# nibox/Pose-Estimation-with-Message-Passing-Networks

Hardware: AMD Instinct MI355X
Metric: images/sec (640px, HRNet-w48) + MPN edge-updates/sec at 1/2/4/8 MI355X (higher is better)
Workload: dtype f16x3; 1 GPU; c3: 8x17x640x640 heatmaps/GPU -> fully graph -> MPN TypeAware-attn T=3; images_per_gpu=8, global_batch=8, persons_per_image=9, nodes_per_gpu=1224, edges_per_gpu=186048, parallelism=image-sharded x1, batches_in_flight=2, detection_and_node_math=fp32

## Files before the change

include/pemp.h:

```cpp
#ifndef PEMP_H_
#define PEMP_H_

#include <stddef.h>
#include <stdint.h>

#ifdef __cplusplus
extern "C" {
#endif

#define PEMP_ABI_VERSION 24

enum {
  PEMP_OK = 0,
  PEMP_ERR_INVALID_ARG = -1,
  PEMP_ERR_HIP = -2,
  PEMP_ERR_WORKSPACE = -3,
  PEMP_ERR_UNSUPPORTED = -4,
};

int pemp_abi_version(void);
const char* pemp_last_error(void);
int pemp_device_check(void);

enum { PEMP_DETECT_NMS = 1, PEMP_DETECT_SELECT = 2, PEMP_DETECT_ALL = 3 };
// ... 174 lines not shown
  const float* edge_img;
  const uint16_t* emb_comp_bf;
  const float* emb_comp_b;
} pemp_mpn_weights;

typedef struct pemp_mpn_desc {
  int32_t num_types;
  int32_t num_joints;
  int32_t steps;
  int32_t aux_loss_steps;
  int32_t aggr;
  int32_t hidden;
  int32_t edge_attr_dim;
  int32_t node_in_dim;
  int32_t precision;
  int32_t types_stride;
  int32_t flags;
} pemp_mpn_desc;

#define PEMP_MPN_PREPARED 1
#define PEMP_MPN_TWO_LAUNCH_FIRST 4
#define PEMP_MPN_FUSED_FIRST_PROFILED 8
#define PEMP_MPN_SEPARATE_PRELUDE 16

size_t pemp_mpn_workspace_size(const pemp_mpn_desc* desc, int64_t N, int64_t E);
size_t pemp_mpn_fused_first_lds_bytes(void);
int pemp_mpn_prelude_grids(int64_t N, int64_t E, int B, int T, int nmax, int edge_grid, int cus, int32_t* out8);
int pemp_mpn_forward(const pemp_mpn_desc* desc, const pemp_mpn_weights* weights, const float* x,
                     const float* edge_attr, const int64_t* edge_index, const int64_t* node_types,
                     int64_t N, int64_t E, float* edge_logits, float* node_logits, float* class_logits,
                     void* workspace, size_t workspace_bytes, void* stream);

int pemp_mpn_forward_fully(const pemp_mpn_desc* desc, const pemp_mpn_weights* weights, const float* x,
                           const float* edge_attr, const int64_t* edge_index, const int64_t* node_types,
                           int64_t N, int64_t E, const int64_t* node_off, const int64_t* node_off_host, int B,
                           float* edge_logits, float* node_logits, float* class_logits,
                           void* workspace, size_t workspace_bytes, void* stream);

int pemp_mpn_forward_fully_cap(const pemp_mpn_desc* desc, const pemp_mpn_weights* weights, const float* x,
                               const float* edge_attr, const int64_t* node_types, int64_t n_cap, int64_t e_cap,
                               const int32_t* n_det, int det_cap, const int64_t* node_off, int B,
                               float* edge_logits, float* node_logits, float* class_logits,
                               void* workspace, size_t workspace_bytes, void* stream);

enum {
  PEMP_STEP_DET = 0, PEMP_STEP_DSC, PEMP_STEP_NDET, PEMP_STEP_X, PEMP_STEP_JDET, PEMP_STEP_JSC, PEMP_STEP_BIDX,
  PEMP_STEP_JTAGS, PEMP_STEP_EIDX, PEMP_STEP_EATTR, PEMP_STEP_NOFF, PEMP_STEP_LOGITS, PEMP_STEP_NOUT
};
typedef struct pemp_step_plan {
  int32_t B, J, H, W, pool_kernel, use_threshold, topk, det_cap, projected;
// ... 99 lines not shown
```

pose-estimation-with-message-passing-networks_amd/_lib.py:

```python
import ctypes
import threading
import os

LIB_PATH = os.environ.get("PEMP_LIB") or os.path.join(os.path.dirname(os.path.abspath(__file__)), "csrc",
                                                     "libpemp.so")
ABI_VERSION = 24

ERR_INVALID_ARG, ERR_HIP, ERR_WORKSPACE, ERR_UNSUPPORTED = -1, -2, -3, -4
MPN_PREPARED, MPN_TWO_LAUNCH_FIRST, MPN_FUSED_FIRST_PROFILED = 1, 4, 8
MPN_SEPARATE_PRELUDE = 16

c_i32, c_i64, c_f32, c_sz, c_p = ctypes.c_int32, ctypes.c_int64, ctypes.c_float, ctypes.c_size_t, ctypes.c_void_p


class PempLayer(ctypes.Structure):
    _fields_ = [("w", c_p), ("b", c_p), ("in_dim", c_i32), ("out_dim", c_i32), ("relu", c_i32), ("pad_", c_i32)]


class PempMlp(ctypes.Structure):
    _fields_ = [("layer", PempLayer * 4), ("n_layers", c_i32), ("pad_", c_i32)]


class PempMpnWeights(ctypes.Structure):
    _fields_ = [("node_emb", PempMlp), ("edge_emb", PempMlp),
                ("pre_w", c_p), ("pre_b", c_p), ("q0_w", c_p), ("q0_b", c_p), ("e1_w", c_p),
                ("e2_w", c_p), ("e2_b", c_p), ("msg_w", c_p), ("attn_w", c_p), ("upd_w", c_p), ("upd_b", c_p),
                ("edge_head", PempMlp), ("node_head", PempMlp), ("class_head", PempMlp),
                ("attn_b", c_f32), ("pad_", c_i32),
                ("e1_bf", c_p), ("e2_bf", c_p), ("msg_bf", c_p), ("head_bf", c_p), ("emb_bf", c_p),
                ("upd_bf", c_p), ("pre_bf", c_p), ("node_img", c_p), ("attn_bv", c_p),
                ("upd_mlp", PempMlp),
                ("ept_l1_w", c_p), ("ept_l1_b", c_p), ("ept_l2_w", c_p), ("ept_l2_b", c_p), ("ept_o1_w", c_p),
                ("ept_o2_w", c_p), ("edge_img", c_p), ("emb_comp_bf", c_p), ("emb_comp_b", c_p)]
# ... 42 lines not shown
                                           c_i64, c_i64, c_f32, c_i32, c_p, c_p, c_p, c_p, c_p, c_p, c_p, c_p, c_p]),
    "pemp_fully_graph": (c_i32, [c_p, c_p, c_i32, c_i64, c_p, c_p]),
    "pemp_knn_workspace_size": (c_sz, [c_p, c_i32]),
    "pemp_knn_graph_build": (c_i32, [c_p, c_p, c_p, c_i32, c_i32, c_p, c_sz, c_i64, c_p, c_p, c_p, c_i32, c_p,
                                     c_i32, c_f32, c_i32, c_p, c_p]),
    "pemp_feature_knn_workspace_size": (c_sz, [c_p, c_i32]),
    "pemp_knn_rows_layout": (c_i32, [c_p, c_i32, c_i32, c_p]),
    "pemp_feature_knn_graph_build": (c_i32, [c_p, c_i32, c_p, c_p, c_p, c_i32, c_i32, c_p, c_sz, c_i64, c_p, c_p,
                                             c_p, c_i32, c_p, c_i32, c_f32, c_i32, c_p, c_p]),
    "pemp_score_graph_workspace_size": (c_sz, [c_p, c_i32, c_i32]),
    "pemp_score_graph": (c_i32, [c_p, c_p, c_p, c_i32, c_i32, c_i64, c_p, c_sz, c_p, c_p]),
    "pemp_gather_projected": (c_i32, [c_p, c_p, c_p, c_i32, c_i32, c_i32, c_i32, c_f32, c_p, c_p, c_i64, c_p, c_p]),
    "pemp_gather_projected_conv": (c_i32, [c_p, c_p, c_p, c_i32, c_i32, c_p, c_p, c_i32, c_i32, c_i32, c_i32, c_i32,
                                           c_f32, c_p, c_p, c_i64, c_p, c_p]),
    "pemp_detect_projected": (c_i32, [c_p, c_p, c_i32, c_i32, c_i32, c_i32, c_i32, c_f32, c_i32, c_i32, c_i32, c_p,
                                      c_sz, c_p, c_p, c_p, c_i32, c_p, c_p]),
    "pemp_gather_projected_tags": (c_i32, [c_p, c_i32, c_i32, c_i32, c_i32, c_p, c_p, c_i64, c_p, c_p]),
    "pemp_project_maps": (c_i32, [c_p, c_i32, c_i32, c_i32, c_i32, c_i32, c_p, c_p, c_p]),
    "pemp_stage_merge": (c_i32, [c_p, c_i32, c_i32, c_i32, c_p, c_i32, c_i32, c_i32, c_i32, c_i32, c_p, c_p]),
    "pemp_edge_features": (c_i32, [c_p, c_p, c_i32, c_p, c_p, c_i64, c_i32, c_f32, c_i32, c_p, c_p]),
    "pemp_mpn_workspace_size": (c_sz, [ctypes.POINTER(PempMpnDesc), c_i64, c_i64]),
    "pemp_mpn_fused_first_lds_bytes": (c_sz, []),
    "pemp_mpn_prelude_grids": (c_i32, [c_i64, c_i64, c_i32, c_i32, c_i32, c_i32, c_i32, c_p]),
    "pemp_mpn_forward": (c_i32, [ctypes.POINTER(PempMpnDesc), ctypes.POINTER(PempMpnWeights), c_p, c_p, c_p, c_p,
                                 c_i64, c_i64, c_p, c_p, c_p, c_p, c_sz, c_p]),
    "pemp_mpn_forward_fully": (c_i32, [ctypes.POINTER(PempMpnDesc), ctypes.POINTER(PempMpnWeights), c_p, c_p, c_p,
                                       c_p, c_i64, c_i64, c_p, c_p, c_i32, c_p, c_p, c_p, c_p, c_sz, c_p]),
    "pemp_mpn_forward_fully_cap": (c_i32, [ctypes.POINTER(PempMpnDesc), ctypes.POINTER(PempMpnWeights), c_p, c_p,
                                           c_p, c_i64, c_i64, c_p, c_i32, c_p, c_i32, c_p, c_p, c_p, c_p, c_sz, c_p]),
    "pemp_mpn_graph_stats": (c_i32, [c_p]),
    "pemp_edge_cus_policy": (c_i32, [c_i32, c_i64, c_i32]),
    "pemp_abi_struct_size": (c_sz, [c_i32]),
    "pemp_mpn_forward_sym": (c_i32, [ctypes.POINTER(PempMpnDesc), ctypes.POINTER(PempMpnWeights), c_p, c_p, c_p,
                                     c_p, c_i64, c_i64, c_p, c_p, c_p, c_p, c_sz, c_p]),
    "pemp_mpn_forward_knn": (c_i32, [ctypes.POINTER(PempMpnDesc), ctypes.POINTER(PempMpnWeights), c_p, c_p, c_p,
                                     c_p, c_i64, c_i64, c_p, c_p, c_p, c_p, c_p, c_i32, c_p, c_p, c_p, c_p, c_sz,
                                     c_p]),
    "pemp_mpn_prepare": (c_i32, [ctypes.POINTER(PempMpnDesc), c_p, c_p, c_i64, c_i64, c_p, c_sz, c_p]),
    "pemp_mpn_order_layout": (c_i32, [ctypes.POINTER(PempMpnDesc), c_i64, c_i64, c_p]),
    "pemp_mpn_edge_image_floats": (c_sz, [ctypes.POINTER(PempMpnDesc), ctypes.POINTER(PempMpnWeights)]),
    "pemp_mpn_edge_image": (c_i32, [ctypes.POINTER(PempMpnDesc), ctypes.POINTER(PempMpnWeights), c_p, c_sz, c_p]),
    "pemp_mpn_node_image_floats": (c_sz, [ctypes.POINTER(PempMpnWeights)]),
    "pemp_mpn_node_image": (c_i32, [ctypes.POINTER(PempMpnWeights), c_p, c_sz, c_p]),
    "pemp_mpn_status": (c_i32, [ctypes.POINTER(PempMpnDesc), c_i64, c_i64, c_p, c_p]),
    "pemp_pose_edge_weights": (c_i32, [c_p, c_i64, c_p, c_p, c_f32, c_i32, c_p, c_i32, c_i64, c_i32, c_p, c_p, c_p,
                                       c_p]),
# ... 121 lines not shown
```

pose-estimation-with-message-passing-networks_amd/csrc/mpn.hip:

```cpp
#include <limits.h>

#include <algorithm>
#include <atomic>
#include <type_traits>
#include <map>
#include <mutex>
#include <string>
#include <vector>
#include <string.h>
#include <math.h>

#include "pemp_common.h"

namespace pemp {
namespace {

constexpr int D = 64;
constexpr int LDW = 72;
constexpr int MAXT = 17;
constexpr int EDGE_WAVES = 16;
constexpr int EMB_WAVES = 16, EMB_PER_CU = 1;
constexpr int EMB_MIN_WAVES_EU = EMB_WAVES * EMB_PER_CU / 4 > 1 ? EMB_WAVES * EMB_PER_CU / 4 : 1;
constexpr int RESERVE_CUS_DEFAULT = 64;
constexpr int64_t RESERVE_MIN_EDGES = 65536;
// ... 2441 lines not shown
          }
        }
    }
  }
}

__global__ __launch_bounds__(256) void node_rows_kernel(NodeRowsArgs a) {
  extern __shared__ __attribute__((aligned(16))) float lds[];
  node_rows_role(a, lds, blockIdx.x);
}

struct NodeTableArgs {
  const float* X;
  int64_t N;
  const float *pre_w, *pre_b;
  const uint16_t* pre_bf;
  int NO, groups;
  float* NT;
  const int64_t* ne;
  const float* agg;
  const int* seg;
  int T;
  const float* upd_b;
};

constexpr int64_t NODE_SUM_TABLE_MAX_MB = 16;
constexpr int TBL_TILES = 2;

template <int PREC, int TILES, bool SUM>
__device__ __forceinline__ void node_table_role(const NodeTableArgs& a, float* xs, int bx) {
  static_assert(!SUM || TILES == 1, "the summing variant takes one 16-node tile per workgroup");
  const int lane = threadIdx.x & 63, wave = threadIdx.x >> 6, c = lane & 15, g = lane >> 4;
  const int chunk = bx / a.groups, grp = bx - chunk * a.groups;
  const int64_t n0 = (int64_t)chunk * 16 * TILES, N = a.ne ? a.ne[0] : a.N;
  if (n0 >= N) return;
  const int nob = a.NO / 16, ob = grp * 4 + wave, obc = min(ob, nob - 1);
  float4 w[8];
  bf16x8_t wh[4], wlo[4];
  f16x8_t fh[4], flo[4];
  if (PREC == 0) {
#pragma unroll
    for (int mb = 0; mb < 8; ++mb) w[mb] = ld4(a.pre_w + (int64_t)(16 * obc + c) * 128 + 16 * mb + 4 * g);
  } else {
#pragma unroll
    for (int kb = 0; kb < 4; ++kb) {
      const int64_t o = (int64_t)(16 * obc + c) * 128 + 32 * kb + 8 * g;
      if (PREC == 1) {
        const __bf16* Wb = reinterpret_cast<const __bf16*>(a.pre_bf);
        wh[kb] = *reinterpret_cast<const bf16x8_t*>(Wb + o);
        wlo[kb] = *reinterpret_cast<const bf16x8_t*>(Wb + (int64_t)a.NO * 128 + o);
      } else {
        const _Float16* Wh = reinterpret_cast<const _Float16*>(a.pre_bf);
        fh[kb] = *reinterpret_cast<const f16x8_t*>(Wh + o);
        flo[kb] = *reinterpret_cast<const f16x8_t*>(Wh + (int64_t)a.NO * 128 + o);
      }
    }
  }
  const float4 bb = ld4(a.pre_b + 16 * obc + 4 * g);
  if constexpr (SUM) {
    const int r = threadIdx.x >> 4, q = threadIdx.x & 15;
    const int64_t n = n0 + r, nc = n < N ? n : N - 1;
    const int T = a.T;
    const float4 x0 = ld4(a.X + nc * 128 + 4 * q);
    float4 y[MAXT];
    int s0[MAXT], s1[MAXT];
#pragma unroll
    for (int t = 0; t < MAXT; ++t) {
      const int tc = min(t, T - 1);
      y[t] = ld4(a.agg + (nc * T + tc) * D + 4 * q);
      s0[t] = a.seg[tc * N + nc];
      s1[t] = a.seg[tc * N + nc + 1];
    }
    float4 v = ld4(a.upd_b + 4 * q);
#pragma unroll
    for (int t = 0; t < MAXT; ++t) {
      if (t < T && s1[t] > s0[t]) { v.x += y[t].x; v.y += y[t].y; v.z += y[t].z; v.w += y[t].w; }
    }
    v = make_float4(fmaxf(v.x, 0.f), fmaxf(v.y, 0.f), fmaxf(v.z, 0.f), fmaxf(v.w, 0.f));
    *reinterpret_cast<float4*>(&xs[r * RS + 4 * q]) = x0;
    *reinterpret_cast<float4*>(&xs[r * RS + 64 + 4 * q]) = v;
    if (grp == 0 && n < N) *reinterpret_cast<float4*>(const_cast<float*>(a.X) + n * 128 + 64 + 4 * q) = v;
  } else {
    float4 t[2 * TILES];
#pragma unroll
    for (int k = 0; k < 2 * TILES; ++k) {
      const int idx = threadIdx.x + 256 * k, row = idx >> 5, c4 = (idx & 31) * 4;
      const int64_t nn = min(n0 + row, N - 1);
      t[k] = ld4(a.X + nn * 128 + c4);
    }
    __builtin_amdgcn_sched_barrier(0);
#pragma unroll
    for (int k = 0; k < 2 * TILES; ++k) {
      const int idx = threadIdx.x + 256 * k, row = idx >> 5, c4 = (idx & 31) * 4;
      *reinterpret_cast<float4*>(&xs[row * RS + c4]) = t[k];
    }
  }
  __syncthreads();
  if (ob >= nob) return;
#pragma unroll
  for (int tile = 0; tile < TILES; ++tile) {
    const int64_t nn = n0 + 16 * tile + c;
    if (n0 + 16 * tile >= N) break;
    float x[8][4];
#pragma unroll
    for (int mb = 0; mb < 8; ++mb) {
// ... 36 lines not shown
#pragma unroll
        for (int kb = 0; kb < 2; ++kb) {
          uint32_t hw[4], lw[4];
#pragma unroll
          for (int d = 0; d < 4; ++d)
            split_pair(xh[2 * kb + (d >> 1)][2 * (d & 1)], xh[2 * kb + (d >> 1)][2 * (d & 1) + 1], ss, hw[d], lw[d]);
          const u32x4_t hv = {hw[0], hw[1], hw[2], hw[3]}, lv = {lw[0], lw[1], lw[2], lw[3]};
          hi[kb] = __builtin_bit_cast(f16x8_t, hv);
          lo[kb] = __builtin_bit_cast(f16x8_t, lv);
        }
#pragma unroll
        for (int kb = 0; kb < 2; ++kb) {
          acc = __builtin_amdgcn_mfma_f32_16x16x32_f16(flo[2 * h + kb], hi[kb], acc, 0, 0, 0);
          acc = __builtin_amdgcn_mfma_f32_16x16x32_f16(fh[2 * h + kb], lo[kb], acc, 0, 0, 0);
          acc = __builtin_amdgcn_mfma_f32_16x16x32_f16(fh[2 * h + kb], hi[kb], acc, 0, 0, 0);
        }
      }
      if (big) acc *= 1.0f / ss;
    }
    if (nn < N) st4(a.NT + nn * a.NO + 16 * ob + 4 * g, acc[0], acc[1], acc[2], acc[3]);
  }
}

template <int PREC, int TILES = TBL_TILES, bool SUM = false>
__global__ __launch_bounds__(256) void node_table_kernel(NodeTableArgs a) {
  __shared__ __attribute__((aligned(16))) float xs[16 * TILES * RS];
  node_table_role<PREC, TILES, SUM>(a, xs, blockIdx.x);
}

template <int PREC>
__global__ __launch_bounds__(256) void prelude_b_kernel(EdgeRangesArgs ra, NodeTableArgs ta, int split) {
  __shared__ __attribute__((aligned(16))) float xs[16 * TBL_TILES * RS];
  const int bx = blockIdx.x;
  if (bx < split) edge_ranges_role(ra, bx);
  else node_table_role<PREC, TBL_TILES, false>(ta, xs, bx - split);
}

static int grid1d(int64_t total, int block, int cap = 65536) {
  int64_t g = (total + block - 1) / block;
  return (int)(g < 1 ? 1 : (g > cap ? cap : g));
}

static bool published_head(const pemp_mlp& m) {
  return m.n_layers == 3 && m.layer[0].in_dim == 64 && m.layer[0].out_dim == 64 && m.layer[0].relu &&
         m.layer[1].in_dim == 64 && m.layer[1].out_dim == 32 && m.layer[1].relu && m.layer[2].in_dim == 32 &&
         m.layer[2].out_dim == 1 && !m.layer[2].relu;
}

template <int AGG, int PREC, int UPD, int STAGE>
static void launch_edge_step_s(const EdgeStepArgs& a, bool head, bool pub, int grid, hipStream_t st) {
  if (!head)
    hipLaunchKernelGGL((edge_step_kernel<AGG, 0, PREC, UPD, STAGE>), dim3(grid), dim3(64 * edge_waves<0>()), 0, st, a);
  else if (pub)
    hipLaunchKernelGGL((edge_step_kernel<AGG, 1, PREC, UPD, STAGE>), dim3(grid), dim3(64 * edge_waves_s<1, STAGE>()), 0,
                       st, a);
  else
    hipLaunchKernelGGL((edge_step_kernel<AGG, 2, PREC, UPD, STAGE>), dim3(grid), dim3(64 * edge_waves<2>()), 0, st, a);
}
// ... 865 lines not shown
  int rows_blocks;
  int a_split;
  int ranges_rb, ranges_blocks;
  int table_blocks;
  int b_split;
};

static PreludeGrids prelude_grids(int64_t N, int64_t E, int B, int T, int nmax, int G, int cus) {
  PreludeGrids g{};
  g.prep_gx = (int)std::max<int64_t>(1, std::min<int64_t>(64, ((int64_t)T * nmax * FULLY_PARTS + 511) / 512));
  g.rows_blocks = (int)((N + 15) / 16);
  g.a_gx = B > 0 ? std::max(1, std::min(g.prep_gx, (cus - g.rows_blocks) / B)) : g.prep_gx;
  g.a_split = g.a_gx * B;
  if (E > 0) {
    g.ranges_rb = std::min(64, (G * (EDGE_WAVES + 12) + 255) / 256);
    g.ranges_blocks = g.ranges_rb + (int)std::min<int64_t>(1024, (E + 255) / 256);
  }
  const int groups = ((128 + 64 * T) / 16 + 3) / 4;
  g.table_blocks = (int)(((N + 16 * TBL_TILES - 1) / (16 * TBL_TILES)) * groups);
  g.b_split = g.ranges_blocks;
  return g;
}

struct ForwardPlan {
  int T, J, steps, aux;
  int64_t tstride;
  bool upd_fused;
  bool pub_head;
  bool ept;
  bool emb_lds, emb_generic, comp, fixed;
  int emb_prec;
  EmbedLayout emb_lo;
  bool fused_heads, fused_embed;
  int edge_grid;
  int NO, table_prec, table_groups;
  unsigned node_grid, table_grid, table_grid1;
  int node_mode;
  bool sum_in_table;
  bool fused_first;
  PreludeGrids grids;
  bool paired;
};

static ForwardPlan plan_forward(const ForwardCall& c) {
  const pemp_mpn_desc& d = *c.desc;
  const pemp_mpn_weights& w = *c.w;
  const int64_t N = c.N, E = c.E;
  ForwardPlan p{};
  p.T = d.num_types; p.J = d.num_joints; p.steps = d.steps; p.aux = d.aux_loss_steps;
  p.tstride = d.types_stride > 0 ? d.types_stride : 1;
  p.upd_fused = edge_upd_fused(d, w);
  p.pub_head = edge_pub_head(d, w);
  p.ept = w.ept_l1_w != nullptr;
  p.emb_lds = mlp_ok(w.edge_emb, 64, 64);
  p.emb_prec = embed_prec(d, w);
  p.emb_lo = embed_layout(w.edge_emb, p.emb_prec);
  p.emb_generic = p.emb_lds && !embed_fixed_shape(p.emb_prec == PEMP_PREC_FP32
                                                      ? embed_layout(w.edge_emb, PEMP_PREC_F16X3)
                                                      : p.emb_lo);
  p.fixed = embed_fixed_shape(p.emb_lo);
  p.comp = embed_composed(p.emb_lo, p.emb_prec, w);
  p.fused_heads = node_heads_fused(w);
  p.fused_embed = node_embed_fused(w);
  p.edge_grid = std::max(edge_cus(E), p.T);
  p.NO = 128 + 64 * p.T;
  p.table_prec = d.precision != PEMP_PREC_FP32 && w.pre_bf ? d.precision : PEMP_PREC_FP32;
  p.table_groups = (p.NO / 16 + 3) / 4;
  p.grids = prelude_grids(N, E, c.order.kind == EdgeOrder::FULLY ? c.order.B : 0, p.T, c.order.nmax, p.edge_grid,
                          num_cus());
  p.node_grid = (unsigned)p.grids.rows_blocks;
  p.table_grid = (unsigned)p.grids.table_blocks;
  p.table_grid1 = (unsigned)(((N + 15) / 16) * p.table_groups);
  p.node_mode = p.upd_fused ? ROWS_SUM : (w.upd_w || w.upd_mlp.n_layers > 0) ? NODE_UPDATE_MLP : ROWS_COPY;
  p.sum_in_table = !p.ept && N * p.T * 256 * (int64_t)p.table_groups <= NODE_SUM_TABLE_MAX_MB << 20;
  p.fused_first = E > 0 && p.steps >= 2 && p.steps - p.aux - 1 > 0 && !(d.flags & PEMP_MPN_TWO_LAUNCH_FIRST) &&
                  d.precision == PEMP_PREC_F16X3 && d.aggr == PEMP_AGGR_ATTN && p.upd_fused && !p.ept &&
                  p.emb_lds && p.comp && w.edge_img &&
                  prof_repeat("edge_step") == 1 &&
                  (!prof_active() || (d.flags & PEMP_MPN_FUSED_FIRST_PROFILED));
  p.paired = c.order.kind == EdgeOrder::FULLY && !(d.flags & (PEMP_MPN_PREPARED | PEMP_MPN_SEPARATE_PRELUDE)) &&
             p.fused_embed && p.steps >= 1 && !prof_active();
  return p;
}

struct Forward {
  const ForwardCall& c;
  const ForwardPlan& p;
  const MpnWs ws;
  const hipStream_t st;
  const int64_t* ne = nullptr;
  const float* node_img = nullptr;
  const float* eimg = nullptr;
  float* r_cur;
  float* r_next;
  int rec = 0;

  Forward(const ForwardCall& call, const ForwardPlan& plan)
// ... 137 lines not shown

  int launch_paired() {
    const PreludeGrids& g = p.grids;
    const FullyPrepArgs fa = fully_args();
    const NodeRowsArgs na = rows_args(ROWS_EMBED, -1, false);
    hipLaunchKernelGGL(prelude_a_kernel, dim3((unsigned)(g.a_split + g.rows_blocks)), dim3(256),
                       prelude_a_lds_bytes(na), st, fa, na, g.a_split, g.a_gx);
    PEMP_LAUNCH_CHECK();
    const EdgeRangesArgs ra = ranges_args();
    const NodeTableArgs ta = table_args();
    with_prec(p.table_prec, [&](auto P) {
      hipLaunchKernelGGL(prelude_b_kernel<decltype(P)::value>, dim3((unsigned)(g.b_split + g.table_blocks)), dim3(256),
                         0, st, ra, ta, g.b_split);
    });
    PEMP_LAUNCH_CHECK();
    return PEMP_OK;
  }

  int node_step(int mode, bool table, int slot, bool dup) {
    const pemp_mpn_weights& w = *c.w;
    const int64_t N = c.N;
    const int T = p.T, J = p.J;
    if (mode == ROWS_SUM && table && slot < 0 && p.sum_in_table) {
      NodeTableArgs ta{ws.X, N, w.pre_w, w.pre_b, w.pre_bf, p.NO, p.table_groups, ws.NT, ne, ws.agg, ws.seg, T,
                       w.upd_b};
      ProfScope prof("node_update_table", st);
      with_prec(p.table_prec, [&](auto P) {
        hipLaunchKernelGGL((node_table_kernel<decltype(P)::value, 1, true>), dim3(p.table_grid1), dim3(256), 0, st, ta);
      });
      PEMP_LAUNCH_CHECK();
      return PEMP_OK;
    }
    if (mode == NODE_UPDATE_MLP && w.upd_mlp.n_layers > 0) {
      NodeMlpArgs ma{ws.agg, ws.seg, T, N, w.upd_mlp, nmlp_max_out(w.upd_mlp), ws.X, ne};
      ProfScope prof("node_update", st);
      hipLaunchKernelGGL(node_mlp_kernel, dim3(p.node_grid), dim3(256), nmlp_lds_bytes(T, w.upd_mlp), st, ma);
      PEMP_LAUNCH_CHECK();
      mode = ROWS_NONE;
    } else if (mode == NODE_UPDATE_MLP) {
      NodeUpdateArgs ua{ws.agg, ws.seg, T, N, w.upd_w, w.upd_b, ws.X, ne};
      ProfScope prof("node_update", st);
      hipLaunchKernelGGL(node_update_kernel, dim3(p.node_grid, 4), dim3(64 * UPD_WAVES), 0, st, ua);
      PEMP_LAUNCH_CHECK();
      mode = ROWS_NONE;
    }
    const NodeRowsArgs na = rows_args(mode, slot, dup);
    if (na.mode != ROWS_NONE || na.node_out) {
      ProfScope prof(mode == ROWS_EMBED ? "node_embed" : "node_update", st);
      hipLaunchKernelGGL(node_rows_kernel, dim3(p.node_grid), dim3(256), node_rows_lds_bytes(na), st, na);
      PEMP_LAUNCH_CHECK();
    }
// ... 379 lines not shown
                        as_stream(stream));
}

extern "C" int pemp_mpn_order_layout(const pemp_mpn_desc* desc, int64_t N, int64_t E, size_t* offs) {
  PEMP_CHECK_ARG(desc && offs && desc->num_types >= 1 && desc->num_types <= MAXT, "pemp_mpn_order_layout: bad desc");
  PEMP_CHECK_ARG(N >= 0 && E >= 0, "pemp_mpn_order_layout: N=%lld E=%lld out of range", (long long)N, (long long)E);
  mpn_carve(nullptr, desc->num_types, N, E, nullptr, offs);
  return PEMP_OK;
}

extern "C" size_t pemp_mpn_fused_first_lds_bytes(void) { return edge_first_lds_bytes(); }

extern "C" int pemp_mpn_prelude_grids(int64_t N, int64_t E, int B, int T, int nmax, int edge_grid, int cus,
                                      int32_t* out8) {
  PEMP_CHECK_ARG(out8 && N >= 0 && E >= 0 && B >= 0 && B <= FULLY_MAXB && T >= 1 && T <= MAXT && nmax >= 0 &&
                     nmax <= FULLY_MAXN && edge_grid >= 1 && cus >= 1,
                 "pemp_mpn_prelude_grids: bad args");
  const PreludeGrids g = prelude_grids(N, E, B, T, nmax, edge_grid, cus);
  static_assert(sizeof(PreludeGrids) == 8 * sizeof(int32_t), "eight ints");
  memcpy(out8, &g, sizeof(g));
  return PEMP_OK;
}

extern "C" size_t pemp_mpn_edge_image_floats(const pemp_mpn_desc* desc, const pemp_mpn_weights* w) {
  if (!desc || !w || desc->num_types < 1 || desc->num_types > MAXT) return 0;
  if (!mlp_ok(w->edge_emb, 64, 64)) return edge_image_base_floats(*desc, *w);
  return embed_image_offset(*desc, *w) + embed_image_floats(embed_layout(w->edge_emb, embed_prec(*desc, *w)));
}

extern "C" int pemp_mpn_edge_image(const pemp_mpn_desc* desc, const pemp_mpn_weights* w, float* image, size_t floats,
                                   void* stream) {
  PEMP_CHECK_ARG(desc && w && image, "pemp_mpn_edge_image: null pointer");
  PEMP_CHECK_ARG(desc->num_types >= 1 && desc->num_types <= MAXT, "pemp_mpn_edge_image: bad num_types");
  PEMP_CHECK_ARG(desc->precision == PEMP_PREC_FP32 || (w->e1_bf && w->e2_bf && w->msg_bf),
                 "pemp_mpn_edge_image: split precisions need the *_bf packs");
  PEMP_CHECK_ARG(w->e1_w && w->e2_w && w->e2_b && w->msg_w, "pemp_mpn_edge_image: null layer weights");
  PEMP_CHECK_ARG(desc->aggr != PEMP_AGGR_ATTN || w->attn_w, "pemp_mpn_edge_image: attention needs attn_w");
  const size_t need = pemp_mpn_edge_image_floats(desc, w);
  PEMP_CHECK_ARG(floats >= need, "pemp_mpn_edge_image: image needs %zu floats", need);
  EdgeImgArgs ia = edge_image_args(*desc, *w, edge_upd_fused(*desc, *w), edge_pub_head(*desc, *w), image);
  hipLaunchKernelGGL(edge_image_kernel, dim3(16, (unsigned)desc->num_types), dim3(256), 0, as_stream(stream), ia);
  PEMP_LAUNCH_CHECK();
  if (mlp_ok(w->edge_emb, 64, 64)) {
    const int prec = embed_prec(*desc, *w);
    const EmbedLayout lo = embed_layout(w->edge_emb, prec);
    float* eimg = image + embed_image_offset(*desc, *w);
// ... 52 lines not shown
```

pose-estimation-with-message-passing-networks_amd/mpn/model.py:

```python
import ctypes
import itertools
import os
import warnings

import numpy as np
import torch
import torch.nn as nn

from .. import _lib
from .fold import F16RangeError, fold_weights
from .edge_type import TypeAwareEdgeUpdate
from .hierarch import HierarchUpdateCnn, HierarchUpdateMlp

_VALIDATE = os.environ.get("PEMP_VALIDATE", "0") not in ("", "0")
_DEBUG_SYNC = os.environ.get("PEMP_DEBUG_SYNC", "0") not in ("", "0")
_FULLY_OFF = os.environ.get("PEMP_NO_FULLY_PREPARE", "0") not in ("", "0")
_SYM_OFF = os.environ.get("PEMP_NO_SYM_PREPARE", "0") not in ("", "0")
_KNN_OFF = os.environ.get("PEMP_NO_KNN_PREPARE", "0") not in ("", "0")
_EDGE_LIMIT = (1 << 23) - 1

AGGR_CODES = {"attn": 0, "add": 1, "sum": 1, "mean": 2, "max": 3}
PRECISIONS = {"fp32": 0, "bf16x3": 1, "f16x3": 2}


def default_precision(aggr_code):
    env = os.environ.get("PEMP_PRECISION", "")
    if env:
        if env not in PRECISIONS:
            raise ValueError(f"PEMP_PRECISION={env!r}: expected one of {sorted(PRECISIONS)}")
        return env
    return "f16x3"
TYPE_LUTS = {"left_right": [0, 1, 1, 2, 2, 3, 3, 4, 4, 5, 5, 6, 6, 7, 7, 8, 8],
             "per_body_part": [0, 0, 0, 0, 0, 1, 1, 2, 3, 2, 3, 4, 5, 4, 5, 4, 5]}


def _rows(logits, n):
    L = logits.shape[1]
    if L != 1:
        return list((logits if logits.shape[0] == n else logits[:n]).unbind(0))
    return [logits[r].view(L, 1).squeeze() for r in range(n)]

# ... 148 lines not shown
        self.node_classification = _make_mlp(64, config.NODE_CLASS.OUTPUT_SIZES, bn=config.BN)
        self.classification = _make_mlp(64, config.CLASS.OUTPUT_SIZES, bn=config.BN)
        self.edge_steps = config.STEPS
        self.node_steps = config.NODE_STEPS
        self.aux_loss_steps = config.AUX_LOSS_STEPS
        self.num_joints = config.CLASS.OUTPUT_SIZES[-1]
        if self.node_steps != 0:
            raise NotImplementedError("NODE_STEPS > 0 (the reference calls the layer without node_types)")
        if config.AGGR_TYPE == "per_type":
            aggr = "attn" if config.AGGR_SUB in ("node_edge_attn", "node_edge_attn_per_type") else config.AGGR
        else:
            aggr = config.AGGR
        if aggr not in AGGR_CODES:
            raise NotImplementedError(f"AGGR={aggr}")
        self.aggr_code = AGGR_CODES[aggr]
        self.precision = default_precision(self.aggr_code)
        self._folded = None
        self._folded_key = None
        self._tensors = None
        self._ws = _lib.Workspace()
        self._desc_ent = None
        self.fuse_first_pass = None
        self.paired_prelude = True
        self.fused_edge_update = False
        self._cap_ok = True
        self._edge_limit = _EDGE_LIMIT
        self._node_rows_limit = _EDGE_LIMIT

    def _apply(self, fn, *args, **kwargs):
        self._tensors = None
        self._folded = None
        return super()._apply(fn, *args, **kwargs)

    def _load_from_state_dict(self, *args, **kwargs):
        self._tensors = None
        return super()._load_from_state_dict(*args, **kwargs)

    def _weights(self, device):
        if self._tensors is None:
            self._tensors = list(self.parameters()) + list(self.buffers())
        key = (device, self.precision, [t._version for t in self._tensors])
        if self._folded is None or self._folded_key != key:
            try:
                self._folded = fold_weights(self, device, self.precision)
            except F16RangeError as exc:
                warnings.warn(f"{exc}; this model runs in precision 'fp32'")
                self.precision = "fp32"
                key = (device, self.precision, key[2])
                self._folded = fold_weights(self, device, self.precision)
            self._folded_key = key
        return self._folded

    def _first_flag(self):
        f = self.fuse_first_pass
        first = 0 if f is None else _lib.MPN_FUSED_FIRST_PROFILED if f else _lib.MPN_TWO_LAUNCH_FIRST
        return first | (0 if self.paired_prelude else _lib.MPN_SEPARATE_PRELUDE)

    def _descriptor(self, A, C, t_stride):
        dkey = (A, C, self.precision, t_stride, self.fuse_first_pass, self.paired_prelude)
        ent = self._desc_ent
        if ent is None or ent[0] != dkey:
            steps, aux = self.edge_steps, self.aux_loss_steps
            self._n_rec = sum(1 for i in range(steps) if i >= steps - aux - 1)
            desc = _lib.PempMpnDesc(self.num_types, self.num_joints, steps, aux, self.aggr_code, 64, A, C,
                                    PRECISIONS[self.precision], t_stride, self._first_flag())
            ent = self._desc_ent = (dkey, ctypes.byref(desc))
        return ent[1]

    _desc_ref = property(lambda self: self._desc_ent[1])
    _desc = property(lambda self: self._desc_ent[1]._obj)

    def _forward_blocks(self, x, edge_attr, edge_index, node_types, kwargs):
        dev = x.device
        N, E = x.shape[0], edge_index.shape[1]
        ei = edge_index.long()
        lo = torch.minimum(ei[0], ei[1])
        blocks = node_blocks(ei, N, self._edge_limit, self._node_rows_limit // self.num_types)
        n_rec = sum(1 for i in range(self.edge_steps) if i >= self.edge_steps - self.aux_loss_steps - 1)
        edge_logits = torch.empty(max(n_rec, 1), E, dtype=torch.float32, device=dev)
        node_logits = torch.empty(n_rec + 1, N, dtype=torch.float32, device=dev)
        class_logits = torch.empty(n_rec + 1, N, self.num_joints, dtype=torch.float32, device=dev)
        sub_kw = {k: v for k, v in kwargs.items() if k == "validate"}
# ... 178 lines not shown
```

Baseline: 36530 images/s.

## Add dedicated node-sum table kernel with weight prefetch and split precision fragments

Replaces the SUM variant of the node table role with a dedicated kernel. It sums per-type aggregates, builds the split hi/lo precision fragments once into LDS, then loops over several output groups per workgroup while prefetching the next group's weight fragment. A grid planner picks tiles per workgroup and groups per run so the grid still covers the CUs, and the segment-emptiness checks are turned into a ballot bitmask. Env flags can force the fused or separate node step. This cuts redundant per-node aggregate loads and fragment conversions across output groups, at the cost of more register and LDS pressure and fewer workgroups.

```diff
diff --git a/include/pemp.h b/include/pemp.h
--- a/include/pemp.h
+++ b/include/pemp.h
@@ -220,10 +220,13 @@
 #define PEMP_MPN_TWO_LAUNCH_FIRST 4
 #define PEMP_MPN_FUSED_FIRST_PROFILED 8
 #define PEMP_MPN_SEPARATE_PRELUDE 16
+#define PEMP_MPN_SEPARATE_NODE_STEP 32
+#define PEMP_MPN_FUSED_NODE_STEP 64
 
 size_t pemp_mpn_workspace_size(const pemp_mpn_desc* desc, int64_t N, int64_t E);
 size_t pemp_mpn_fused_first_lds_bytes(void);
 int pemp_mpn_prelude_grids(int64_t N, int64_t E, int B, int T, int nmax, int edge_grid, int cus, int32_t* out8);
+int pemp_mpn_node_step_grid(int64_t N, int T, int cus, int32_t* out4);
 int pemp_mpn_forward(const pemp_mpn_desc* desc, const pemp_mpn_weights* weights, const float* x,
                      const float* edge_attr, const int64_t* edge_index, const int64_t* node_types,
                      int64_t N, int64_t E, float* edge_logits, float* node_logits, float* class_logits,
diff --git a/pose-estimation-with-message-passing-networks_amd/_lib.py b/pose-estimation-with-message-passing-networks_amd/_lib.py
--- a/pose-estimation-with-message-passing-networks_amd/_lib.py
+++ b/pose-estimation-with-message-passing-networks_amd/_lib.py
@@ -9,6 +9,7 @@
 ERR_INVALID_ARG, ERR_HIP, ERR_WORKSPACE, ERR_UNSUPPORTED = -1, -2, -3, -4
 MPN_PREPARED, MPN_TWO_LAUNCH_FIRST, MPN_FUSED_FIRST_PROFILED = 1, 4, 8
 MPN_SEPARATE_PRELUDE = 16
+MPN_SEPARATE_NODE_STEP, MPN_FUSED_NODE_STEP = 32, 64
 
 c_i32, c_i64, c_f32, c_sz, c_p = ctypes.c_int32, ctypes.c_int64, ctypes.c_float, ctypes.c_size_t, ctypes.c_void_p
 
@@ -97,6 +98,7 @@
     "pemp_mpn_workspace_size": (c_sz, [ctypes.POINTER(PempMpnDesc), c_i64, c_i64]),
     "pemp_mpn_fused_first_lds_bytes": (c_sz, []),
     "pemp_mpn_prelude_grids": (c_i32, [c_i64, c_i64, c_i32, c_i32, c_i32, c_i32, c_i32, c_p]),
+    "pemp_mpn_node_step_grid": (c_i32, [c_i64, c_i32, c_i32, c_p]),
     "pemp_mpn_forward": (c_i32, [ctypes.POINTER(PempMpnDesc), ctypes.POINTER(PempMpnWeights), c_p, c_p, c_p, c_p,
                                  c_i64, c_i64, c_p, c_p, c_p, c_p, c_sz, c_p]),
     "pemp_mpn_forward_fully": (c_i32, [ctypes.POINTER(PempMpnDesc), ctypes.POINTER(PempMpnWeights), c_p, c_p, c_p,
diff --git a/pose-estimation-with-message-passing-networks_amd/csrc/mpn.hip b/pose-estimation-with-message-passing-networks_amd/csrc/mpn.hip
--- a/pose-estimation-with-message-passing-networks_amd/csrc/mpn.hip
+++ b/pose-estimation-with-message-passing-networks_amd/csrc/mpn.hip
@@ -2487,65 +2487,64 @@
   const int* seg;
   int T;
   const float* upd_b;
+  int runs, G;
 };
 
 constexpr int64_t NODE_SUM_TABLE_MAX_MB = 16;
 constexpr int TBL_TILES = 2;
 
-template <int PREC, int TILES, bool SUM>
+template <int PREC>
+struct TableFrag {
+  u32x4_t hi[4], lo[4];
+  float4 bb;
+};
+template <>
+struct TableFrag<0> {
+  float4 w[8];
+  float4 bb;
+};
+
+template <int PREC>
+__device__ __forceinline__ TableFrag<PREC> table_frag_load(const NodeTableArgs& a, int ob, int c, int g) {
+  TableFrag<PREC> f;
+  if constexpr (PREC == 0) {
+#pragma unroll
+    for (int mb = 0; mb < 8; ++mb) f.w[mb] = ld4(a.pre_w + (int64_t)(16 * ob + c) * 128 + 16 * mb + 4 * g);
+  } else {
+#pragma unroll
+    for (int kb = 0; kb < 4; ++kb) {
+      const uint16_t* o = a.pre_bf + (int64_t)(16 * ob + c) * 128 + 32 * kb + 8 * g;
+      f.hi[kb] = *reinterpret_cast<const u32x4_t*>(o);
+      f.lo[kb] = *reinterpret_cast<const u32x4_t*>(o + (int64_t)a.NO * 128);
+    }
+  }
+  f.bb = ld4(a.pre_b + 16 * ob + 4 * g);
+  return f;
+}
+
+template <int PREC, int TILES>
 __device__ __forceinline__ void node_table_role(const NodeTableArgs& a, float* xs, int bx) {
-  static_assert(!SUM || TILES == 1, "the summing variant takes one 16-node tile per workgroup");
   const int lane = threadIdx.x & 63, wave = threadIdx.x >> 6, c = lane & 15, g = lane >> 4;
   const int chunk = bx / a.groups, grp = bx - chunk * a.groups;
   const int64_t n0 = (int64_t)chunk * 16 * TILES, N = a.ne ? a.ne[0] : a.N;
   if (n0 >= N) return;
   const int nob = a.NO / 16, ob = grp * 4 + wave, obc = min(ob, nob - 1);
+  const TableFrag<PREC> f = table_frag_load<PREC>(a, obc, c, g);
   float4 w[8];
   bf16x8_t wh[4], wlo[4];
   f16x8_t fh[4], flo[4];
-  if (PREC == 0) {
-#pragma unroll
-    for (int mb = 0; mb < 8; ++mb) w[mb] = ld4(a.pre_w + (int64_t)(16 * obc + c) * 128 + 16 * mb + 4 * g);
+  if constexpr (PREC == 0) {
+#pragma unroll
+    for (int mb = 0; mb < 8; ++mb) w[mb] = f.w[mb];
   } else {
 #pragma unroll
     for (int kb = 0; kb < 4; ++kb) {
-      const int64_t o = (int64_t)(16 * obc + c) * 128 + 32 * kb + 8 * g;
-      if (PREC == 1) {
-        const __bf16* Wb = reinterpret_cast<const __bf16*>(a.pre_bf);
-        wh[kb] = *reinterpret_cast<const bf16x8_t*>(Wb + o);
-        wlo[kb] = *reinterpret_cast<const bf16x8_t*>(Wb + (int64_t)a.NO * 128 + o);
-      } else {
-        const _Float16* Wh = reinterpret_cast<const _Float16*>(a.pre_bf);
-        fh[kb] = *reinterpret_cast<const f16x8_t*>(Wh + o);
-        flo[kb] = *reinterpret_cast<const f16x8_t*>(Wh + (int64_t)a.NO * 128 + o);
-      }
-    }
-  }
-  const float4 bb = ld4(a.pre_b + 16 * obc + 4 * g);
-  if constexpr (SUM) {
-    const int r = threadIdx.x >> 4, q = threadIdx.x & 15;
-    const int64_t n = n0 + r, nc = n < N ? n : N - 1;
-    const int T = a.T;
-    const float4 x0 = ld4(a.X + nc * 128 + 4 * q);
-    float4 y[MAXT];
-    int s0[MAXT], s1[MAXT];
-#pragma unroll
-    for (int t = 0; t < MAXT; ++t) {
-      const int tc = min(t, T - 1);
-      y[t] = ld4(a.agg + (nc * T + tc) * D + 4 * q);
-      s0[t] = a.seg[tc * N + nc];
-      s1[t] = a.seg[tc * N + nc + 1];
-    }
-    float4 v = ld4(a.upd_b + 4 * q);
-#pragma unroll
-    for (int t = 0; t < MAXT; ++t) {
-      if (t < T && s1[t] > s0[t]) { v.x += y[t].x; v.y += y[t].y; v.z += y[t].z; v.w += y[t].w; }
-    }
-    v = make_float4(fmaxf(v.x, 0.f), fmaxf(v.y, 0.f), fmaxf(v.z, 0.f), fmaxf(v.w, 0.f));
-    *reinterpret_cast<float4*>(&xs[r * RS + 4 * q]) = x0;
-    *reinterpret_cast<float4*>(&xs[r * RS + 64 + 4 * q]) = v;
-    if (grp == 0 && n < N) *reinterpret_cast<float4*>(const_cast<float*>(a.X) + n * 128 + 64 + 4 * q) = v;
-  } else {
+      wh[kb] = __builtin_bit_cast(bf16x8_t, f.hi[kb]); wlo[kb] = __builtin_bit_cast(bf16x8_t, f.lo[kb]);
+      fh[kb] = __builtin_bit_cast(f16x8_t, f.hi[kb]); flo[kb] = __builtin_bit_cast(f16x8_t, f.lo[kb]);
+    }
+  }
+  const float4 bb = f.bb;
+  {
     float4 t[2 * TILES];
 #pragma unroll
     for (int k = 0; k < 2 * TILES; ++k) {
@@ -2628,18 +2627,164 @@
   }
 }
 
-template <int PREC, int TILES = TBL_TILES, bool SUM = false>
+template <int PREC, int TILES = TBL_TILES>
 __global__ __launch_bounds__(256) void node_table_kernel(NodeTableArgs a) {
   __shared__ __attribute__((aligned(16))) float xs[16 * TILES * RS];
-  node_table_role<PREC, TILES, SUM>(a, xs, blockIdx.x);
-}
-
+  node_table_role<PREC, TILES>(a, xs, blockIdx.x);
+}
+
+template <int PREC, int TILES>
+__global__ __launch_bounds__(256) __attribute__((amdgpu_waves_per_eu(PREC == 1 && TILES == 2 ? 4 : 5)))
+void node_sum_table_kernel(NodeTableArgs a) {
+  static_assert(TILES == 1 || TILES == 2, "one split unit (tile, half) per wave");
+  static_assert(MAXT <= 32, "non-empty segments of a row as one bit mask");
+  __shared__ __attribute__((aligned(16))) float xs[16 * TILES * RS];
+  __shared__ float xscale[TILES * 64];
+  static_assert(TILES * 2 * 4 * 64 * 4 <= 16 * TILES * RS, "the fragments fit over the rows");
+  const int lane = threadIdx.x & 63, wave = __builtin_amdgcn_readfirstlane(threadIdx.x >> 6), c = lane & 15, g = lane >> 4;
+  const int item = blockIdx.x / a.runs, run = blockIdx.x - item * a.runs;
+  const int64_t n0 = (int64_t)item * 16 * TILES, N = a.ne ? a.ne[0] : a.N;
+  if (n0 >= N) return;
+  const int nob = a.NO / 16, ng = min(a.G, a.groups - run * a.G), T = a.T;
+  int ob = run * a.G * 4 + wave;
+  {
+    const int r = threadIdx.x >> 4, q = threadIdx.x & 15;
+#pragma unroll 1
+    for (int tile = 0; tile < TILES; ++tile) {
+      const int64_t n = n0 + 16 * tile + r, nc = n < N ? n : N - 1;
+      const float4 x0 = ld4(a.X + nc * 128 + 4 * q);
+      const char* aggb = reinterpret_cast<const char*>(a.agg);
+      const uint32_t voff = ((uint32_t)nc * (uint32_t)T * D + 4u * q) * (uint32_t)sizeof(float);
+      float4 y[MAXT];
+#pragma unroll
+      for (int t = 0; t < MAXT; ++t)
+        y[t] = ld4(reinterpret_cast<const float*>(aggb + (size_t)min(t, T - 1) * (D * sizeof(float)) + voff));
+      const int tq = min(q, T - 1);
+      const bool has = a.seg[tq * N + nc + 1] > a.seg[tq * N + nc];
+      uint32_t full = (uint32_t)(__ballot(has) >> (16 * g)) & 0xffffu;
+#pragma unroll
+      for (int t = 16; t < MAXT; ++t) {
+        const int tc = min(t, T - 1);
+        if (a.seg[tc * N + nc + 1] > a.seg[tc * N + nc]) full |= 1u << t;
+      }
+      float4 v = ld4(a.upd_b + 4 * q);
+#pragma unroll
+      for (int t = 0; t < MAXT; ++t) {
+        if (t < T && (full >> t & 1u)) { v.x += y[t].x; v.y += y[t].y; v.z += y[t].z; v.w += y[t].w; }
+      }
+      v = make_float4(fmaxf(v.x, 0.f), fmaxf(v.y, 0.f), fmaxf(v.z, 0.f), fmaxf(v.w, 0.f));
+      *reinterpret_cast<float4*>(&xs[(16 * tile + r) * RS + 4 * q]) = x0;
+      *reinterpret_cast<float4*>(&xs[(16 * tile + r) * RS + 64 + 4 * q]) = v;
+      if (run == 0 && n < N) *reinterpret_cast<float4*>(const_cast<float*>(a.X) + n * 128 + 64 + 4 * q) = v;
+    }
+  }
+  TableFrag<PREC> cur = table_frag_load<PREC>(a, min(ob, nob - 1), c, g);
+  __syncthreads();
+  u32x4_t* const frag = reinterpret_cast<u32x4_t*>(xs);
+  if constexpr (PREC != 0) {
+    const int ut = wave >> 1, uh = wave & 1;
+    const bool unit = wave < 2 * TILES;
+    u32x4_t fr[4] = {};
+    float ss = 1.0f;
+    if (unit) {
+      float xh[4][4], xo[4][4];
+#pragma unroll
+      for (int mb = 0; mb < 4; ++mb) {
+        const float4 v = ld4(&xs[(16 * ut + c) * RS + 64 * uh + 16 * mb + 4 * g]);
+        const float4 o = ld4(&xs[(16 * ut + c) * RS + 64 * (1 - uh) + 16 * mb + 4 * g]);
+        xh[mb][0] = v.x; xh[mb][1] = v.y; xh[mb][2] = v.z; xh[mb][3] = v.w;
+        xo[mb][0] = o.x; xo[mb][1] = o.y; xo[mb][2] = o.z; xo[mb][3] = o.w;
+      }
+      if constexpr (PREC == 1) {
+        bf16x8_t hi[2], lo[2];
+        split_bf16(xh, hi, lo);
+#pragma unroll
+        for (int kb = 0; kb < 2; ++kb) {
+          fr[2 * kb] = __builtin_bit_cast(u32x4_t, hi[kb]);
+          fr[2 * kb + 1] = __builtin_bit_cast(u32x4_t, lo[kb]);
+        }
+      } else {
+        const float mx = fmaxf(frag_absmax(xh), frag_absmax(xo));
+        const bool big = __any(!(mx < F16_BIG));
+        ss = big ? f16_item_scale(mx, 1.0f) : 1.0f;
+#pragma unroll
+        for (int kb = 0; kb < 2; ++kb) {
+          uint32_t hw[4], lw[4];
+#pragma unroll
+          for (int d = 0; d < 4; ++d)
+            split_pair(xh[2 * kb + (d >> 1)][2 * (d & 1)], xh[2 * kb + (d >> 1)][2 * (d & 1) + 1], ss, hw[d], lw[d]);
+          fr[2 * kb] = u32x4_t{hw[0], hw[1], hw[2], hw[3]};
+          fr[2 * kb + 1] = u32x4_t{lw[0], lw[1], lw[2], lw[3]};
+        }
+      }
+    }
+    __syncthreads();
+    if (unit) {
+#pragma unroll
+      for (int k = 0; k < 4; ++k) frag[((ut * 2 + uh) * 4 + k) * 64 + lane] = fr[k];
+      if (PREC == 2 && uh == 0) xscale[ut * 64 + lane] = ss;
+    }
+    __syncthreads();
+  }
+  const uint32_t nt_lane = (uint32_t)(c * a.NO + 4 * g);
+#pragma unroll 1
+  for (int gi = 0; gi < ng; ++gi, ob += 4) {
+    TableFrag<PREC> nxt = cur;
+    if (gi + 1 < ng) nxt = table_frag_load<PREC>(a, min(ob + 4, nob - 1), c, g);
+    if (ob < nob) {
+#pragma unroll
+      for (int tile = 0; tile < TILES; ++tile) {
+        const int64_t nn = n0 + 16 * tile + c;
+        if (n0 + 16 * tile >= N) break;
+        f32x4 acc = {cur.bb.x, cur.bb.y, cur.bb.z, cur.bb.w};
+        if constexpr (PREC == 0) {
+#pragma unroll
+          for (int mb = 0; mb < 8; ++mb) {
+            const float4 v = ld4(&xs[(16 * tile + c) * RS + 16 * mb + 4 * g]);
+            acc = mfma4(cur.w[mb].x, v.x, acc);
+            acc = mfma4(cur.w[mb].y, v.y, acc);
+            acc = mfma4(cur.w[mb].z, v.z, acc);
+            acc = mfma4(cur.w[mb].w, v.w, acc);
+          }
+        } else if constexpr (PREC == 1) {
+#pragma unroll
+          for (int h = 0; h < 2; ++h)
+#pragma unroll
+            for (int kb = 0; kb < 2; ++kb) {
+              const bf16x8_t hi = __builtin_bit_cast(bf16x8_t, frag[((tile * 2 + h) * 4 + 2 * kb) * 64 + lane]);
+              const bf16x8_t lo = __builtin_bit_cast(bf16x8_t, frag[((tile * 2 + h) * 4 + 2 * kb + 1) * 64 + lane]);
+              acc = __builtin_amdgcn_mfma_f32_16x16x32_bf16(__builtin_bit_cast(bf16x8_t, cur.lo[2 * h + kb]), hi, acc, 0, 0, 0);
+              acc = __builtin_amdgcn_mfma_f32_16x16x32_bf16(__builtin_bit_cast(bf16x8_t, cur.hi[2 * h + kb]), lo, acc, 0, 0, 0);
+              acc = __builtin_amdgcn_mfma_f32_16x16x32_bf16(__builtin_bit_cast(bf16x8_t, cur.hi[2 * h + kb]), hi, acc, 0, 0, 0);
+            }
+        } else {
+          const float ss = xscale[tile * 64 + lane];
+          const bool big = __any(ss != 1.0f);
+          acc *= 2048.0f * ss;
+#pragma unroll
+          for (int h = 0; h < 2; ++h)
+#pragma unroll
+            for (int kb = 0; kb < 2; ++kb) {
+              const f16x8_t hi = __builtin_bit_cast(f16x8_t, frag[((tile * 2 + h) * 4 + 2 * kb) * 64 + lane]);
+              const f16x8_t lo = __builtin_bit_cast(f16x8_t, frag[((tile * 2 + h) * 4 + 2 * kb + 1) * 64 + lane]);
+              acc = __builtin_amdgcn_mfma_f32_16x16x32_f16(__builtin_bit_cast(f16x8_t, cur.lo[2 * h + kb]), hi, acc, 0, 0, 0);
+              acc = __builtin_amdgcn_mfma_f32_16x16x32_f16(__builtin_bit_cast(f16x8_t, cur.hi[2 * h + kb]), lo, acc, 0, 0, 0);
+              acc = __builtin_amdgcn_mfma_f32_16x16x32_f16(__builtin_bit_cast(f16x8_t, cur.hi[2 * h + kb]), hi, acc, 0, 0, 0);
+            }
+          if (big) acc *= 1.0f / ss;
+        }
+        if (nn < N) st4(a.NT + ((n0 + 16 * tile) * a.NO + 16 * ob) + nt_lane, acc[0], acc[1], acc[2], acc[3]);
+      }
+    }
+    cur = nxt;
+  }
+}
 template <int PREC>
 __global__ __launch_bounds__(256) void prelude_b_kernel(EdgeRangesArgs ra, NodeTableArgs ta, int split) {
   __shared__ __attribute__((aligned(16))) float xs[16 * TBL_TILES * RS];
   const int bx = blockIdx.x;
   if (bx < split) edge_ranges_role(ra, bx);
-  else node_table_role<PREC, TBL_TILES, false>(ta, xs, bx - split);
+  else node_table_role<PREC, TBL_TILES>(ta, xs, bx - split);
 }
 
 static int grid1d(int64_t total, int block, int cap = 65536) {
@@ -3551,6 +3696,24 @@
   return g;
 }
 
+struct NodeStepGrid {
+  int tiles, items, G, runs;
+};
+
+static NodeStepGrid node_step_grid(int64_t N, int groups, int cus) {
+  NodeStepGrid s{};
+  const int64_t wide = (N + 16 * TBL_TILES - 1) / (16 * TBL_TILES);
+  s.tiles = wide * groups >= cus ? TBL_TILES : 1;
+  s.items = (int)((N + 16 * s.tiles - 1) / (16 * s.tiles));
+  s.G = 1;
+  s.runs = groups;
+  for (int runs = 1; runs < groups; ++runs) {
+    const int G = (groups + runs - 1) / runs, r = (groups + G - 1) / G;
+    if ((int64_t)s.items * r >= cus) { s.G = G; s.runs = r; break; }
+  }
+  return s;
+}
+
 struct ForwardPlan {
   int T, J, steps, aux;
   int64_t tstride;
@@ -3563,7 +3726,8 @@
   bool fused_heads, fused_embed;
   int edge_grid;
   int NO, table_prec, table_groups;
-  unsigned node_grid, table_grid, table_grid1;
+  unsigned node_grid, table_grid;
+  NodeStepGrid step_grid;
   int node_mode;
   bool sum_in_table;
   bool fused_first;
@@ -3599,9 +3763,11 @@
                           num_cus());
   p.node_grid = (unsigned)p.grids.rows_blocks;
   p.table_grid = (unsigned)p.grids.table_blocks;
-  p.table_grid1 = (unsigned)(((N + 15) / 16) * p.table_groups);
+  p.step_grid = node_step_grid(N, p.table_groups, num_cus());
   p.node_mode = p.upd_fused ? ROWS_SUM : (w.upd_w || w.upd_mlp.n_layers > 0) ? NODE_UPDATE_MLP : ROWS_COPY;
-  p.sum_in_table = !p.ept && N * p.T * 256 * (int64_t)p.table_groups <= NODE_SUM_TABLE_MAX_MB << 20;
+  p.sum_in_table = !p.ept && !(d.flags & PEMP_MPN_SEPARATE_NODE_STEP) &&
+                   ((d.flags & PEMP_MPN_FUSED_NODE_STEP) ||
+                    N * p.T * 256 * (int64_t)p.step_grid.runs <= NODE_SUM_TABLE_MAX_MB << 20);
   p.fused_first = E > 0 && p.steps >= 2 && p.steps - p.aux - 1 > 0 && !(d.flags & PEMP_MPN_TWO_LAUNCH_FIRST) &&
                   d.precision == PEMP_PREC_F16X3 && d.aggr == PEMP_AGGR_ATTN && p.upd_fused && !p.ept &&
                   p.emb_lds && p.comp && w.edge_img &&
@@ -3785,11 +3951,16 @@
     const int64_t N = c.N;
     const int T = p.T, J = p.J;
     if (mode == ROWS_SUM && table && slot < 0 && p.sum_in_table) {
+      const NodeStepGrid& sg = p.step_grid;
       NodeTableArgs ta{ws.X, N, w.pre_w, w.pre_b, w.pre_bf, p.NO, p.table_groups, ws.NT, ne, ws.agg, ws.seg, T,
-                       w.upd_b};
+                       w.upd_b, sg.runs, sg.G};
+      const dim3 grid((unsigned)(sg.items * sg.runs));
       ProfScope prof("node_update_table", st);
       with_prec(p.table_prec, [&](auto P) {
-        hipLaunchKernelGGL((node_table_kernel<decltype(P)::value, 1, true>), dim3(p.table_grid1), dim3(256), 0, st, ta);
+        if (sg.tiles == 1)
+          hipLaunchKernelGGL((node_sum_table_kernel<decltype(P)::value, 1>), grid, dim3(256), 0, st, ta);
+        else
+          hipLaunchKernelGGL((node_sum_table_kernel<decltype(P)::value, TBL_TILES>), grid, dim3(256), 0, st, ta);
       });
       PEMP_LAUNCH_CHECK();
       return PEMP_OK;
@@ -4215,6 +4386,14 @@
   return PEMP_OK;
 }
 
+extern "C" int pemp_mpn_node_step_grid(int64_t N, int T, int cus, int32_t* out4) {
+  PEMP_CHECK_ARG(out4 && N >= 0 && T >= 1 && T <= MAXT && cus >= 1, "pemp_mpn_node_step_grid: bad args");
+  const NodeStepGrid s = node_step_grid(N, ((128 + 64 * T) / 16 + 3) / 4, cus);
+  static_assert(sizeof(NodeStepGrid) == 4 * sizeof(int32_t), "four ints");
+  memcpy(out4, &s, sizeof(s));
+  return PEMP_OK;
+}
+
 extern "C" size_t pemp_mpn_edge_image_floats(const pemp_mpn_desc* desc, const pemp_mpn_weights* w) {
   if (!desc || !w || desc->num_types < 1 || desc->num_types > MAXT) return 0;
   if (!mlp_ok(w->edge_emb, 64, 64)) return edge_image_base_floats(*desc, *w);
diff --git a/pose-estimation-with-message-passing-networks_amd/mpn/model.py b/pose-estimation-with-message-passing-networks_amd/mpn/model.py
--- a/pose-estimation-with-message-passing-networks_amd/mpn/model.py
+++ b/pose-estimation-with-message-passing-networks_amd/mpn/model.py
@@ -17,6 +17,8 @@
 _FULLY_OFF = os.environ.get("PEMP_NO_FULLY_PREPARE", "0") not in ("", "0")
 _SYM_OFF = os.environ.get("PEMP_NO_SYM_PREPARE", "0") not in ("", "0")
 _KNN_OFF = os.environ.get("PEMP_NO_KNN_PREPARE", "0") not in ("", "0")
+_SEPARATE_NODE_STEP = os.environ.get("PEMP_MPN_SEPARATE_NODE_STEP", "0") not in ("", "0")
+_FUSED_NODE_STEP = os.environ.get("PEMP_MPN_FUSED_NODE_STEP", "0") not in ("", "0")
 _EDGE_LIMIT = (1 << 23) - 1
 
 AGGR_CODES = {"attn": 0, "add": 1, "sum": 1, "mean": 2, "max": 3}
@@ -211,6 +213,7 @@
         self._desc_ent = None
         self.fuse_first_pass = None
         self.paired_prelude = True
+        self.fused_node_step = False if _SEPARATE_NODE_STEP else True if _FUSED_NODE_STEP else None
         self.fused_edge_update = False
         self._cap_ok = True
         self._edge_limit = _EDGE_LIMIT
@@ -243,10 +246,12 @@
     def _first_flag(self):
         f = self.fuse_first_pass
         first = 0 if f is None else _lib.MPN_FUSED_FIRST_PROFILED if f else _lib.MPN_TWO_LAUNCH_FIRST
-        return first | (0 if self.paired_prelude else _lib.MPN_SEPARATE_PRELUDE)
+        n = self.fused_node_step
+        node = 0 if n is None else _lib.MPN_FUSED_NODE_STEP if n else _lib.MPN_SEPARATE_NODE_STEP
+        return first | (0 if self.paired_prelude else _lib.MPN_SEPARATE_PRELUDE) | node
 
     def _descriptor(self, A, C, t_stride):
-        dkey = (A, C, self.precision, t_stride, self.fuse_first_pass, self.paired_prelude)
+        dkey = (A, C, self.precision, t_stride, self._first_flag())
         ent = self._desc_ent
         if ent is None or ent[0] != dkey:
             steps, aux = self.edge_steps, self.aux_loss_steps
```

Result: no change. 36600 images/s (median of 3 runs) (+0.2%).
